# stefanch/sGDML

Measured on AMD Instinct MI355X. Metric: kernel-matrix build+solve wall-clock, N_train=1000 21-atom (aspirin-sized), lower is better.
Workload: dtype f64

## Files before the change

sgdml_amd/csrc/chol.hip:

```cpp
#include "common.h"
#include <type_traits>
#include <utility>

typedef double d4 __attribute__((ext_vector_type(4)));
typedef double d2 __attribute__((ext_vector_type(2)));

#define GT 128
#define GBK 16
#define GPITCH 17

struct GemmArgs {
  const double* A;
  const double* B;
  double* C;
  int64_t M, N, K, lda, ldb, ldc;
  int lower;
  int tiles_m, tiles_n;
  int64_t n_super;
  int64_t s_begin;
  int super_n;
  int aligned;
  int cyc_W, cyc_rank;
  int64_t cyc_lb0, cyc_nb, cyc_col0, cyc_block_rows;
  double* diagA;
  int diag_nbw;
  int64_t diag_off;
  int* diag_info;
  int col0_first;
  int* ready;
  int ready_target, ready_rows;
  const double* A2;
  const double* B2;
  double* C2;
  int64_t M2, N2, K2;
  int tiles2;
};

__global__ void __launch_bounds__(256, 2) gemm_nt_sub_diag_kernel(GemmArgs g);

template <bool FULL>
__device__ __forceinline__ void gemm_load_tile(const double* __restrict__ G, int64_t ld,
                                               int64_t row0, int64_t nrows, int64_t k0, int64_t K,
                                               int tid, d2 (&r)[4]) {
#pragma unroll
  for (int s = 0; s < 4; ++s) {
    int cidx = tid + 256 * s;
    int row = cidx >> 3, kc = (cidx & 7) * 2;
    int64_t gr = row0 + row, gk = k0 + kc;
    if (FULL) {
      r[s] = *reinterpret_cast<const d2*>(G + gr * ld + gk);
    } else {
      int64_t cr = gr < nrows ? gr : nrows - 1;
      int64_t ck0 = gk < K ? gk : K - 1, ck1 = gk + 1 < K ? gk + 1 : K - 1;
      double v0 = G[cr * ld + ck0], v1 = G[cr * ld + ck1];
      d2 v;
      v.x = (gr < nrows && gk < K) ? v0 : 0.0;
      v.y = (gr < nrows && gk + 1 < K) ? v1 : 0.0;
      r[s] = v;
    }
  }
}

__device__ __forceinline__ void gemm_load_tile_g(const double* __restrict__ base, const unsigned (&off)[4], d2 (&r)[4]) {
  typedef const __attribute__((address_space(1))) char* gcptr;
  typedef const __attribute__((address_space(1))) d2* gd2ptr;
  const uint64_t p = reinterpret_cast<uint64_t>(base);
  const uint32_t lo = __builtin_amdgcn_readfirstlane((uint32_t)p), hi = __builtin_amdgcn_readfirstlane((uint32_t)(p >> 32));
  gcptr b = (gcptr)(((uint64_t)hi << 32) | lo);
// ... 130 lines not shown
          const int64_t gr = row0 + wm * 64 + i * 16 + lk + 4 * r;
          if (gc < g.N && gr < g.M) g.C[gr * g.ldc + gc] = -acc[i][j][r];
        }
    }
    return;
  }
#pragma unroll
  for (int j = 0; j < 4; ++j) {
    double cv[4][4];
    const int64_t gc = col0 + wn * 64 + j * 16 + li;
    const bool cok = gc < g.N;
#pragma unroll
    for (int i = 0; i < 4; ++i)
#pragma unroll
      for (int r = 0; r < 4; ++r) {
        const int64_t gr = row0 + wm * 64 + i * 16 + lk + 4 * r;
        const int64_t cr = gr < g.M ? gr : g.M - 1, cc = cok ? gc : g.N - 1;
        cv[i][r] = g.C[cr * g.ldc + cc];
      }
#pragma unroll
    for (int i = 0; i < 4; ++i)
#pragma unroll
      for (int r = 0; r < 4; ++r) {
        const int64_t gr = row0 + wm * 64 + i * 16 + lk + 4 * r;
        if (cok && gr < g.M) g.C[gr * g.ldc + gc] = cv[i][r] - acc[i][j][r];
      }
  }
}

template <bool OW>
__device__ __forceinline__ void gemm_block(const GemmArgs& g, double (*lds)[2][GT * GPITCH], int64_t b) {
  if (b < g.tiles2) {
    const int tn2 = (int)((g.N2 + GT - 1) / GT);
    const int64_t ti = b / tn2, tj = b - ti * tn2;
    if (ti < tn2 && tj > ti) return;
    GemmArgs h = g;
    h.A = g.A2; h.B = g.B2; h.C = g.C2; h.M = g.M2; h.N = g.N2; h.K = g.K2;
    h.aligned = ((reinterpret_cast<uintptr_t>(g.A2) | reinterpret_cast<uintptr_t>(g.B2)) & 15) == 0 && g.aligned;
    const int64_t row0 = ti * GT, col0 = tj * GT;
    const bool full = (row0 + GT <= h.M) && (col0 + GT <= h.N) && ((h.K & (GBK - 1)) == 0) && h.aligned;
    if (full)
      gemm_tile_body<true, false>(h, lds, row0, col0);
    else
      gemm_tile_body<false, false>(h, lds, row0, col0);
    if (g.ready && ti < g.ready_rows && tj < g.ready_rows) {
      __threadfence();
      __syncthreads();
      if (threadIdx.x == 0) atomicAdd(g.ready, 1);
    }
    return;
  }
  b -= g.tiles2;
  const int64_t xcd = b & 7, loc = b >> 3;
  const int64_t s = g.s_begin + (loc >> 6) * 8 + xcd;
  const int within = (int)(loc & 63);
  if (s >= g.n_super) return;
  int64_t SI, SJ;
  if (g.lower) {
    int64_t sr = s, shift = 0;
    const int64_t sm = (g.tiles_m + 7) / 8;
    if (g.col0_first) {
      if (s < sm) { SI = s; SJ = 0; sr = -1; }
      else { sr = s - sm; shift = 1; }
    }
    if (sr >= 0) {
      SI = (int64_t)((sqrt(8.0 * (double)sr + 1.0) - 1.0) * 0.5);
      while (SI * (SI + 1) / 2 > sr) --SI;
      while ((SI + 1) * (SI + 2) / 2 <= sr) ++SI;
      SJ = sr - SI * (SI + 1) / 2;
      SI += shift; SJ += shift;
    }
  } else {
    SI = s / g.super_n;
    SJ = s - SI * g.super_n;
  }
  const int64_t ti = SI * 8 + (within >> 3), tj = SJ * 8 + (within & 7);
  if (ti >= g.tiles_m || tj >= g.tiles_n) return;
  if (g.lower && tj > ti) return;
  const int64_t row0 = ti * GT, col0 = tj * GT;
  if (g.cyc_W > 0 && row0 + GT <= g.cyc_block_rows) {
    const int64_t gb = (g.cyc_lb0 + row0 / g.cyc_nb) * g.cyc_W + g.cyc_rank;
    const int64_t grow_last = gb * g.cyc_nb + (row0 + GT - 1) % g.cyc_nb;
    if (g.cyc_col0 + col0 > grow_last) return;
  }
  const bool full = (row0 + GT <= g.M) && (col0 + GT <= g.N) && ((g.K & (GBK - 1)) == 0) && g.aligned;
  if (full)
    gemm_tile_body<true, OW>(g, lds, row0, col0);
  else
    gemm_tile_body<false, OW>(g, lds, row0, col0);
  if (g.ready && g.tiles2 == 0 && ti < g.ready_rows && tj < g.ready_rows) {
    __threadfence();
    __syncthreads();
    if (threadIdx.x == 0) atomicAdd(g.ready, 1);
  }
}

__global__ void __launch_bounds__(256, 2) gemm_nt_sub_kernel(GemmArgs g) {
  __shared__ __attribute__((aligned(16))) double lds[2][2][GT * GPITCH];
  gemm_block<false>(g, lds, blockIdx.x);
}


__global__ void __launch_bounds__(256, 2) gemm_nt_neg_kernel(GemmArgs g) {
  __shared__ __attribute__((aligned(16))) double lds[2][2][GT * GPITCH];
  gemm_block<true>(g, lds, blockIdx.x);
}

struct DiagJob {
  double* A = nullptr;
  int nbw = 0;
  int64_t off = 0;
  int* ready = nullptr;
  int ready_target = 0;
  bool col0_first = false;
  const double* A2 = nullptr;
  const double* B2 = nullptr;
  double* C2 = nullptr;
  int64_t M2 = 0, N2 = 0, K2 = 0;
};

static int launch_gemm_nt_sub_part(gdml_ctx* ctx, hipStream_t st, const double* A, int64_t lda,
                                   const double* B, int64_t ldb, double* C, int64_t ldc, int64_t M,
                                   int64_t N, int64_t K, int lower, double f0, double f1, bool timed,
                                   const DiagJob* diag = nullptr, const CyclicLower* cyc = nullptr, bool overwrite = false) {
  if (M <= 0 || N <= 0 || K <= 0) return GDML_OK;
  GemmArgs g;
  g.A = A; g.B = B; g.C = C; g.M = M; g.N = N; g.K = K; g.lda = lda; g.ldb = ldb; g.ldc = ldc;
  g.lower = lower;
  g.diagA = nullptr; g.diag_nbw = 0; g.diag_off = 0; g.diag_info = nullptr;
  g.cyc_W = 0; g.cyc_rank = 0; g.cyc_lb0 = 0; g.cyc_nb = 0; g.cyc_col0 = 0; g.cyc_block_rows = 0;
  g.col0_first = (diag && diag->col0_first) ? 1 : 0;
  g.ready = nullptr; g.ready_target = 0; g.ready_rows = 0;
  g.A2 = g.B2 = nullptr; g.C2 = nullptr; g.M2 = g.N2 = g.K2 = 0; g.tiles2 = 0;
  if (cyc) { g.cyc_W = cyc->W; g.cyc_rank = cyc->rank; g.cyc_lb0 = cyc->lb0; g.cyc_nb = cyc->nb; g.cyc_col0 = cyc->col0; g.cyc_block_rows = cyc->block_rows; }
  g.aligned = ((reinterpret_cast<uintptr_t>(A) | reinterpret_cast<uintptr_t>(B)) & 15) == 0 &&
              (lda % 2 == 0) && (ldb % 2 == 0);
  g.tiles_m = (int)((M + GT - 1) / GT);
  g.tiles_n = (int)((N + GT - 1) / GT);
  int64_t sm = (g.tiles_m + 7) / 8, sn = (g.tiles_n + 7) / 8;
  g.super_n = (int)sn;
  const int64_t n_super_all = lower ? sm * (sm + 1) / 2 : sm * sn;
  g.s_begin = (int64_t)(f0 * (double)n_super_all);
  g.n_super = (f1 >= 1.0) ? n_super_all : (int64_t)(f1 * (double)n_super_all);
  const bool has_diag = diag && diag->A;
  if (g.n_super <= g.s_begin) {
    if (!has_diag) return GDML_OK;
    g.n_super = g.s_begin;
  }
  int64_t groups = (g.n_super - g.s_begin + 7) / 8;
  int64_t blocks = groups * 512;
  const int slot = (timed && st == (ctx->kt_stream ? ctx->kt_stream : ctx->stream)) ? ktime_begin(ctx) : -1;
  if (has_diag) {
    g.diagA = diag->A; g.diag_nbw = diag->nbw; g.diag_off = diag->off; g.diag_info = ctx->d_info;
    if (diag->ready) { g.ready = diag->ready; g.ready_target = diag->ready_target; g.ready_rows = diag->nbw * 64 / GT; }
    if (diag->A2 && diag->M2 > 0) {
      g.A2 = diag->A2; g.B2 = diag->B2; g.C2 = diag->C2; g.M2 = diag->M2; g.N2 = diag->N2; g.K2 = diag->K2;
      g.tiles2 = (int)(ceil_div(g.M2, GT) * ceil_div(g.N2, GT));
    }
    hipLaunchKernelGGL(gemm_nt_sub_diag_kernel, dim3((unsigned)(blocks + 1 + g.tiles2)), dim3(256), 0, st, g);
  } else if (overwrite)
    hipLaunchKernelGGL(gemm_nt_neg_kernel, dim3((unsigned)blocks), dim3(256), 0, st, g);
  else
    hipLaunchKernelGGL(gemm_nt_sub_kernel, dim3((unsigned)blocks), dim3(256), 0, st, g);
  const double part = (double)(g.n_super - g.s_begin) / (double)n_super_all;
  ktime_end(ctx, slot, has_diag ? "gemm_nt_sub_diag" : "gemm_nt_sub",
            part * (lower ? (double)M * (double)(M + 1) * (double)K : 2.0 * (double)M * (double)N * (double)K) +
                2.0 * (double)g.M2 * (double)g.N2 * (double)g.K2);
  ctx->launch_counter++;
  HIP_CHECK(ctx, hipGetLastError());
  return GDML_OK;
}

int launch_gemm_nt_sub(gdml_ctx* ctx, hipStream_t st, const double* A, int64_t lda,
                              const double* B, int64_t ldb, double* C, int64_t ldc, int64_t M,
                              int64_t N, int64_t K, int lower) {
  return launch_gemm_nt_sub_part(ctx, st, A, lda, B, ldb, C, ldc, M, N, K, lower, 0.0, 1.0, true);
}

int launch_gemm_nt_neg(gdml_ctx* ctx, hipStream_t st, const double* A, int64_t lda, const double* B, int64_t ldb,
                       double* C, int64_t ldc, int64_t M, int64_t N, int64_t K) {
  return launch_gemm_nt_sub_part(ctx, st, A, lda, B, ldb, C, ldc, M, N, K, 0, 0.0, 1.0, true, nullptr, nullptr, true);
}

int launch_gemm_nt_sub_cyclic(gdml_ctx* ctx, hipStream_t st, const double* A, int64_t lda, const double* B, int64_t ldb,
                              double* C, int64_t ldc, int64_t M, int64_t N, int64_t K, const CyclicLower& cyc) {
  return launch_gemm_nt_sub_part(ctx, st, A, lda, B, ldb, C, ldc, M, N, K, 0, 0.0, 1.0, true, nullptr, &cyc);
}

__device__ __forceinline__ double readlane_f64(double v, int l) {
  const int lo = __builtin_amdgcn_readlane(__double2loint(v), l);
  const int hi = __builtin_amdgcn_readlane(__double2hiint(v), l);
  return __hiloint2double(hi, lo);
}
__device__ __forceinline__ int potrf64_wave(double* T, double* cb , int lane) {
  double row[64];
#pragma unroll
  for (int c = 0; c < 64; ++c) row[c] = T[lane * 65 + c];
  int fail = 0;
#pragma unroll
  for (int jb = 0; jb < 8; ++jb) {
// ... 734 lines not shown
  if (min_rows < 1) min_rows = 1;
  int64_t OB = (int64_t)ctx_opt(ctx, "chol.outer", 1024);
  if (OB != 2 * NB || NB % GT != 0) OB = NB;
  const int64_t outer_min_rows = (int64_t)ctx_opt(ctx, "chol.outer_min_rows", 16384);
  auto width_at = [&](int64_t c0) -> int64_t {
    const int64_t left = n - (c0 + OB);
    const int64_t w = (OB > NB && left > 0 && left >= outer_min_rows) ? OB : NB;
    return (n - c0 < w) ? n - c0 : w;
  };
  int64_t k0 = 0, nb = (n < NB) ? n : NB;
  int ready_count = 0;
  HIP_CHECK(ctx, hipMemsetAsync(ctx->d_info + 6, 0, 2 * sizeof(int), ctx->stream));
  GDML_TRY(panel_factor(ctx, st, A, n_rows, ld, 0, nb));
  for (;;) {
    const int64_t t0 = k0 + nb;
    if (t0 >= n) break;
    const int64_t nb2 = width_at(t0);
    const int64_t t1 = t0 + nb2;
    const double* P = A + t0 * ld + k0;
    const bool fuse = (nb2 % 64 == 0) && (n - t1 >= min_rows) && (n_rows - t1 > 0);
    if (fuse && nb2 == 2 * NB) {
      const int64_t ta = t0 + NB;
      const int64_t sm = (ceil_div(n_rows - t0, GT) + 7) / 8, n_super_all = sm * (sm + 1) / 2;
      int64_t s_split = n_super_all / 2;
      if (s_split < sm) s_split = sm;
      const double fs = ((double)s_split + 0.5) / (double)n_super_all;
      DiagJob dj;
      dj.A = A + t0 * ld + t0; dj.nbw = (int)(NB / 64); dj.off = t0;
      dj.col0_first = true;
      dj.ready = ctx->d_info + 6;
      const int block_tiles = (int)((NB / GT) * (NB / GT + 1) / 2);
      ready_count += block_tiles;
      dj.ready_target = ready_count;
      GDML_TRY(launch_gemm_nt_sub_part(ctx, st, P, ld, P, ld, A + t0 * ld + t0, ld, n_rows - t0, n - t0, nb, 1, 0.0, fs, true,
                                       &dj));
      double* Xa = A + ta * ld + t0;
      GDML_TRY(launch_panel_trsm(ctx, st, A + t0 * ld + t0, Xa, ld, (int)NB, n_rows - ta));
      dj.A = A + ta * ld + ta; dj.off = ta;
      dj.A2 = Xa; dj.B2 = Xa; dj.C2 = A + ta * ld + ta; dj.M2 = n_rows - ta; dj.N2 = NB; dj.K2 = NB;
      ready_count += block_tiles;
      dj.ready_target = ready_count;
      GDML_TRY(launch_gemm_nt_sub_part(ctx, st, P, ld, P, ld, A + t0 * ld + t0, ld, n_rows - t0, n - t0, nb, 1, fs, 1.0, true,
                                       &dj));
      GDML_TRY(launch_panel_trsm(ctx, st, A + ta * ld + ta, A + t1 * ld + ta, ld, (int)NB, n_rows - t1));
    } else {
      GDML_TRY(launch_gemm_nt_sub(ctx, st, P, ld, P, ld, A + t0 * ld + t0, ld, n_rows - t0, nb2, nb, 0));
      const double* P1 = A + t1 * ld + k0;
      if (fuse) {
        DiagJob dj;
        dj.A = A + t0 * ld + t0;
        dj.nbw = (int)(nb2 / 64);
        dj.off = t0;
        GDML_TRY(launch_gemm_nt_sub_part(ctx, st, P1, ld, P1, ld, A + t1 * ld + t1, ld, n_rows - t1, n - t1, nb, 1, 0.0,
                                         1.0, true, &dj));
        GDML_TRY(launch_panel_trsm(ctx, st, A + t0 * ld + t0, A + t1 * ld + t0, ld, (int)nb2, n_rows - t1));
      } else if (t1 < n) {
        hipStream_t sp = ctx->stream2;
        HIP_CHECK(ctx, hipEventRecord(ctx->ev_la[0], st));
        HIP_CHECK(ctx, hipStreamWaitEvent(sp, ctx->ev_la[0], 0));
        GDML_TRY(panel_factor(ctx, sp, A, n_rows, ld, t0, nb2));
        HIP_CHECK(ctx, hipEventRecord(ctx->ev_la[1], sp));
        GDML_TRY(launch_gemm_nt_sub(ctx, st, P1, ld, P1, ld, A + t1 * ld + t1, ld, n_rows - t1, n - t1, nb, 1));
        HIP_CHECK(ctx, hipStreamWaitEvent(st, ctx->ev_la[1], 0));
      } else {
        GDML_TRY(panel_factor(ctx, st, A, n_rows, ld, t0, nb2));
      }
// ... 340 lines not shown
```

sgdml_amd/csrc/common.h:

```cpp
#pragma once
#include <hip/hip_runtime.h>
#include <stdint.h>
#include <stdio.h>
#include <stdlib.h>
#include <string.h>

#include <map>
#include <string>
#include <vector>

#include "../../include/gdml_hip.h"

#define GDML_MAX_ATOMS 4096

struct Lattice {
  double lat[9];
  double inv[9];
  int use;
};

struct PhaseStat {
  double ms = 0.0;
  int64_t launches = 0;
};
// ... 26 lines not shown
  std::vector<int32_t> h_tp, h_perm, h_pinv;
};

struct Model {
  int64_t M = 0;
  int N = 0, D = 0, P = 0;
  double sig = 0;
  double* xp = nullptr;
  double* jap = nullptr;
  double* ja = nullptr;
  double* aE = nullptr;
  int32_t* tp = nullptr;
  bool has_aE = false;
};

enum CtxSlot {
  SLOT_PREDICT_WS = 0,
  SLOT_MATVEC_OUT = 1,
  SLOT_LEV_SCORES = 2,
  SLOT_PRECON_GEMV = 3,
  SLOT_PREDICT_STATS = 4,
  SLOT_PANEL_SAVE = 5,
  SLOT_LU_UT = 6,
  SLOT_WIDE_WS = 7,
  SLOT_PANEL_TRSM = 8,
  SLOT_WIDE_PARTS = 9,
  SLOT_PRECON_MF = 10,
  SLOT_F32_GRAM_ROWS = 11,
  SLOT_MATVEC_VREF = 12,
  SLOT_GRAM_WS = 13,
  SLOT_GRAM_ROWS = 14,
  SLOT_COUNT
};

struct gdml_ctx {
  int device = 0;
  int num_cus = 256;
  hipStream_t stream = nullptr;
  hipStream_t stream2 = nullptr;
  hipStream_t kt_stream = nullptr;
  hipEvent_t ev0 = nullptr, ev1 = nullptr;
  hipEvent_t ev_la[6] = {};
  std::string err;
  std::map<std::string, double> opts;
  int64_t held = 0;
  std::map<void*, int64_t> allocs;
  std::map<std::string, PhaseStat> phases;
  std::string phase_pending;
  int64_t phase_pending_launches = 0;
  double* h_pin = nullptr;
  int64_t h_pin_bytes = 0;
  double* h_map = nullptr;
  double* h_map_dev = nullptr;
  unsigned* d_fused_counter = nullptr;
  unsigned long long fused_seq = 0;
  int64_t launch_counter = 0;
  bool profiling = false;
  std::map<std::string, KernelStat> kstats;
  std::vector<PendingTiming> pending;
  std::vector<hipEvent_t> event_pool;

  TrainSet ts;
  Model model;

  double* K = nullptr;
  int64_t K_rows = 0, K_cols = 0, K_extra = 0, K_ld = 0, K_bytes = 0;
  bool K_factored = false;
  bool K_destroyed = false;
  bool K_is_A = false;
  bool K_rhs_row = false;
  double* d_rhs = nullptr;
  double K_lam = 0, K_sig = 0;
  bool uncert_ready = false;
  int K_use_E = 0;

  double* precon = nullptr;
  int64_t precon_m = 0, precon_n = 0;
  int precon_form = 0, precon_stage = 2, precon_use_E = 0;
  double precon_sig = 0;
  double* precon_Z = nullptr;
  int64_t precon_Z_bytes = 0;
  int64_t* precon_idx = nullptr;
  int64_t precon_idx_bytes = 0;
  float* precon_X32 = nullptr;
  int64_t precon_X32_bytes = 0;
  bool precon_X32_inplace = false;
  int64_t precon_X32_ld = 0;
  std::vector<double> precon_lev_cache;
  double* precon_T0 = nullptr;
  int64_t precon_T0_bytes = 0;

  double* scratch = nullptr;
  int64_t scratch_bytes = 0;
  double* slot[SLOT_COUNT] = {};
  int64_t slot_bytes[SLOT_COUNT] = {};
  int* d_info = nullptr;

  void* comm = nullptr;
  void* comm2 = nullptr;
  int rank = 0, world = 1;
  struct {
    bool on = false;
    void *comm = nullptr, *comm2 = nullptr;
    int rank = 0, world = 1;
    bool virtual_rank = false;
    gdml_host_allreduce ar = nullptr;
    gdml_host_allgather ag = nullptr;
  } parked;
  bool virtual_rank = false;
  gdml_host_allreduce host_allreduce = nullptr;
  bool comm_aborted = false;
  gdml_host_allgather host_allgather = nullptr;
  void* host_coll_user = nullptr;
  double* h_coll = nullptr;
  int64_t h_coll_bytes = 0;
  int64_t coll_calls = 0;
  double coll_bytes = 0.0;
  bool K_sharded = false;
  int64_t K_rows_global = 0;
};

int gdml_fail(gdml_ctx* ctx, int code, const char* fmt, ...);
double ctx_opt(const gdml_ctx* ctx, const char* key, double dflt);
static inline int ctx_opt_i(const gdml_ctx* ctx, const char* key, int dflt) { return (int)ctx_opt(ctx, key, (double)dflt); }

#define HIP_CHECK(ctx, call)                                                              \
  do {                                                                                    \
    hipError_t e__ = (call);                                                              \
    if (e__ != hipSuccess)                                                                \
// ... 36 lines not shown

int desc_device(gdml_ctx* ctx, const double* d_R, int64_t M, int N, const double* lat,
                const double* lat_inv, double* d_x, double* d_g);
int predict_device(gdml_ctx* ctx, const double* d_xq, const double* d_gq, int64_t B, double* d_E,
                   double* d_F);
int hess_device(gdml_ctx* ctx, const double* d_xq, const double* d_gq, int64_t B, double* d_E, double* d_F,
                double* d_H);
int predict_wide_device(gdml_ctx* ctx, const double* d_xq, int64_t B, double* part_F, double* part_E);
int set_alphas_device(gdml_ctx* ctx, const double* d_alphas_F, const double* d_alphas_E);
int matvec_device(gdml_ctx* ctx, double lam, int use_E_cstr, const double* d_v, int64_t n,
                  double* d_out);
int chol_factor_device(gdml_ctx* ctx, double* A, int64_t n, int64_t ld, int* info, int64_t n_rows = 0);
int lu_factor_device(gdml_ctx* ctx, double* A, int64_t n, int64_t ld, int64_t* d_piv, int* info_out);
int chol_solve_device(gdml_ctx* ctx, const double* L, int64_t n, int64_t ld, double* d_b,
                      double* d_z, double* d_x);
int operator_model_from_trainset(gdml_ctx* ctx, double sig);
int launch_gemm_nt_sub(gdml_ctx* ctx, hipStream_t st, const double* A, int64_t lda, const double* B,
                       int64_t ldb, double* C, int64_t ldc, int64_t M, int64_t N, int64_t K, int lower);
int launch_gemm_nt_neg(gdml_ctx* ctx, hipStream_t st, const double* A, int64_t lda, const double* B, int64_t ldb,
                       double* C, int64_t ldc, int64_t M, int64_t N, int64_t K);
struct CyclicLower {
  int W = 0, rank = 0;
  int64_t lb0 = 0, nb = 0, col0 = 0, block_rows = 0;
};
int launch_gemm_nt_sub_cyclic(gdml_ctx* ctx, hipStream_t st, const double* A, int64_t lda, const double* B, int64_t ldb,
                              double* C, int64_t ldc, int64_t M, int64_t N, int64_t K, const CyclicLower& cyc);
int launch_trsm64(gdml_ctx* ctx, hipStream_t st, const double* Ld, double* X, int64_t ld, int w,
                  int64_t m, int64_t ldl = 0);
int launch_panel_trsm(gdml_ctx* ctx, hipStream_t st, const double* L, double* X, int64_t ld, int nb, int64_t m,
                      int64_t ldl = 0);
int panel_factor_steps(gdml_ctx* ctx, hipStream_t st, double* A, int64_t n, int64_t ld, int64_t k0, int64_t nb);
int chol_bwd_device(gdml_ctx* ctx, const double* L, int64_t n, int64_t ld, double* d_z, double* d_x);
int tall_trsm(gdml_ctx* ctx, const double* L, double* X, int64_t n, int64_t m, int64_t ld, int look = -1);
int ctx_slot(gdml_ctx* ctx, int slot, int64_t bytes, double** out);
int ctx_slot_release(gdml_ctx* ctx, int slot);
struct GramSplit {
  int n3, nblk, npairs, S;
  int64_t n, ld, L;
};
GramSplit gram_split(int64_t n, int n3);
static inline int64_t pad_rows128(int64_t rows) { return (rows + 127) / 128 * 128; }
int gram_workspace(gdml_ctx* ctx, const GramSplit& g, const char* chunk_opt, int64_t items, int64_t ws_per_item, int64_t ws_fixed,
                   int64_t* chunk, double** rows, double** ws);
void block_gram_launch(gdml_ctx* ctx, const GramSplit& g, const double* Z, double* part, int64_t items, bool diag, int64_t first0,
                       int64_t first_stride, int64_t pitch = 0);
int cross_rows_launch(gdml_ctx* ctx, const double* xt, const double* gt, int64_t M, const double* xq, const double* gq, int bc,
                      double* rows, int64_t ld, double* kqq, double sgn, double sig, const char* tname);
void cov_reduce_launch(gdml_ctx* ctx, const GramSplit& g, const double* part, const double* nkqq, double* out, int64_t items,
                       int full);
void shard_points(const gdml_ctx* ctx, int64_t M, int64_t* p0, int64_t* p1, int64_t* pts_per);
struct VecLayout {
  int64_t n = 0, n_ff = 0, M = 0, N3 = 0, per = 0;
  int64_t chunk = 0, n_pad = 0, row0 = 0, n_loc = 0;
  int two_seg = 0;
  __host__ __device__ int64_t pos(int64_t g) const {
    if (!two_seg) return g;
    if (g < n_ff) {
      const int64_t pt = g / N3, r = pt / per;
      return r * chunk + (pt - r * per) * N3 + (g - pt * N3);
    }
    const int64_t e = g - n_ff, r = e / per;
    const int64_t cnt = (M - r * per < per) ? M - r * per : per;
    return r * chunk + cnt * N3 + (e - r * per);
  }
};
VecLayout vec_layout(const gdml_ctx* ctx, int use_E_cstr);
// ... 11 lines not shown
```

sgdml_amd/csrc/ctx.hip:

```cpp
#include <stdarg.h>

#include <mutex>

#include "common.h"

static std::string g_create_err;

int gdml_fail(gdml_ctx* ctx, int code, const char* fmt, ...) {
  char buf[1024];
  va_list ap;
  va_start(ap, fmt);
  vsnprintf(buf, sizeof(buf), fmt, ap);
  va_end(ap);
  if (ctx)
    ctx->err = buf;
  else
    g_create_err = buf;
  return code;
}

extern "C" int gdml_abi_version(void) { return 4; }

static const char* kKnownOptions[] = {
    "asm.wave", "asm.j_chunk", "asm.lower", "asm.strip", "asm.i_chunk",
    "asm.pts", "asm.pts_nv", "asm.pts_nt", "asm.pts_xcd", "asm.pts_i_chunk", "asm.pts_debug", "asm.perm_debug", "asm.perm_w", "asm.perm_lds_kb", "asm.perm_level", "asm.perm_nimg", "asm.perm_pg", "asm.perm_na", "asm.perm_fast_store", "asm.perm_i_chunk", "asm.perm_compact", "asm.perm_lds_rows", "asm.big1", "asm.perm2", "asm.perm2_min_n", "asm.perm2_min_p", "asm.perm2_split", "asm.perm2_post", "asm.perm2_ed", "asm.perm2_es", "asm.perm2_direct", "asm.perm2_chunk", "asm.perm2_i_chunk", "asm.perm2_debug",
    "nys.trsm_left", "nys.syrk_split", "predict.wide_pad", "predict.tn_fill", "chol.nb", "pcg.gemv_plain",
    "chol.fused_min_rows", "chol.outer", "chol.outer_min_rows", "trsm.debug",
    "trsv.persist", "predict.wave_only", "predict.mfma", "predict.fill", "predict.mfma_wide", "predict.fused", "predict.fused_rows", "predict.fused_spin",
    "lu.nb", "comm.force_collectives", "nys.force_qr", "nys.force_fail", "dist.nb", "dist.lookahead", "dist.force_panels", "pcg.depth", "pcg.precon_form", "pcg.f32_rows_per", "pcg.f32_rw", "pcg.f32_min_pivot", "pcg.f32_last_min_pivot", "pcg.f32_gram_rows", "pcg.f32_inplace",
    "predict.hess_generic", "predict.hess_chunk_rows", "predict.cov_chunk", "predict.cov_global", "predict.cov_few_rows", "predict.cov_few_split_timers", "chol.loo_chunk", "chol.extend_chunk", "chol.remove_chunk", "chol.select_chunk", "chol.select_mem_budget",
    "chol.evidence_chunk", "chol.evidence_mem_budget", "chol.evidence_global"};

double ctx_opt(const gdml_ctx* ctx, const char* key, double dflt) {
  auto it = ctx->opts.find(key);
  return it == ctx->opts.end() ? dflt : it->second;
}

extern "C" int gdml_set_option(gdml_ctx* ctx, const char* key, double value) {
  if (!ctx || !key) return GDML_ERR_INVALID;
  for (const char* k : kKnownOptions)
    if (strcmp(k, key) == 0) {
      ctx->opts[key] = value;
      return GDML_OK;
    }
  return gdml_fail(ctx, GDML_ERR_INVALID, "gdml_set_option: unknown option '%s'", key);
}

extern "C" int gdml_get_option(gdml_ctx* ctx, const char* key, double* value_out, int* is_set_out) {
  if (!ctx || !key) return GDML_ERR_INVALID;
  auto it = ctx->opts.find(key);
  if (value_out) *value_out = it == ctx->opts.end() ? 0.0 : it->second;
  if (is_set_out) *is_set_out = it != ctx->opts.end();
  return GDML_OK;
}

static void options_from_env(gdml_ctx* ctx) {
  const char* e = getenv("GDML_OPTIONS");
  if (!e) return;
  std::string s(e);
  size_t pos = 0;
// ... 114 lines not shown
      (e = hipEventCreateWithFlags(&ctx->ev_la[1], hipEventDisableTiming)) != hipSuccess ||
      (e = hipEventCreateWithFlags(&ctx->ev_la[2], hipEventDisableTiming)) != hipSuccess ||
      (e = hipEventCreateWithFlags(&ctx->ev_la[3], hipEventDisableTiming)) != hipSuccess ||
      (e = hipEventCreateWithFlags(&ctx->ev_la[4], hipEventDisableTiming)) != hipSuccess ||
      (e = hipEventCreateWithFlags(&ctx->ev_la[5], hipEventDisableTiming)) != hipSuccess ||
      (e = hipMalloc((void**)&ctx->d_info, 64)) != hipSuccess) {
    gdml_fail(nullptr, GDML_ERR_HIP, "context setup failed: %s", hipGetErrorString(e));
    delete ctx;
    return GDML_ERR_HIP;
  }
  options_from_env(ctx);
  *ctx_out = ctx;
  return GDML_OK;
}

extern "C" int gdml_ctx_destroy(gdml_ctx* ctx) {
  if (!ctx) return GDML_OK;
  hipSetDevice(ctx->device);
  hipDeviceSynchronize();
  comm_destroy(ctx);
  for (auto& t : ctx->pending) {
    hipEventDestroy(t.e0);
    hipEventDestroy(t.e1);
  }
  for (auto e : ctx->event_pool) hipEventDestroy(e);
  {
    std::lock_guard<std::mutex> lk(g_arena_mu);
    DeviceArena* a = arena_of(ctx);
    for (auto& kv : ctx->allocs)
      if (!arena_owns(a, kv.first)) hipFree(kv.first);
    ctx->allocs.clear();
    arena_release_owner(ctx);
  }
  if (ctx->d_info) hipFree(ctx->d_info);
  if (ctx->ev0) hipEventDestroy(ctx->ev0);
  if (ctx->ev1) hipEventDestroy(ctx->ev1);
  for (hipEvent_t ev : ctx->ev_la)
    if (ev) hipEventDestroy(ev);
  if (ctx->stream) hipStreamDestroy(ctx->stream);
  if (ctx->stream2) hipStreamDestroy(ctx->stream2);
  if (ctx->h_pin) hipHostFree(ctx->h_pin);
  if (ctx->h_map) hipHostFree(ctx->h_map);
  if (ctx->h_coll) hipHostFree(ctx->h_coll);
  delete ctx;
  return GDML_OK;
}

extern "C" const char* gdml_last_error(const gdml_ctx* ctx) {
  return ctx ? ctx->err.c_str() : g_create_err.c_str();
}

extern "C" int gdml_sync(gdml_ctx* ctx) {
  if (!ctx) return GDML_ERR_INVALID;
  HIP_CHECK(ctx, hipSetDevice(ctx->device));
  HIP_CHECK(ctx, hipStreamSynchronize(ctx->stream));
  HIP_CHECK(ctx, hipStreamSynchronize(ctx->stream2));
  return GDML_OK;
}

extern "C" int gdml_mem_info(gdml_ctx* ctx, int64_t* held, int64_t* free_b, int64_t* total_b) {
  if (!ctx) return GDML_ERR_INVALID;
  size_t f = 0, t = 0;
  HIP_CHECK(ctx, hipSetDevice(ctx->device));
  HIP_CHECK(ctx, hipMemGetInfo(&f, &t));
  if (held) *held = ctx->held;
  {
// ... 271 lines not shown
```

Before: 1.297.

## Balance lower-triangular GEMM tiles across XCDs with host-built schedule tables

Adds a host-built, cached tile schedule for the lower-triangular trailing GEMM update. Full 8x8 super-tiles are decoded arithmetically, and partial or diagonal tiles are dealt evenly across the eight XCD block slots through a small device table. The schedule accounts for second-GEMM lead work and for two-launch splits. It also packs the fused second GEMM's tiles compactly, so no blocks are launched only to exit early on upper-triangle tiles. The aim is to cut wasted empty blocks and XCD load imbalance. The cost is host-side schedule construction, plus a one-time device allocation, copy and stream sync per new shape.

After: 1.281 (median of 6 runs). 1.3% less time.

```diff
diff --git a/sgdml_amd/csrc/chol.hip b/sgdml_amd/csrc/chol.hip
--- a/sgdml_amd/csrc/chol.hip
+++ b/sgdml_amd/csrc/chol.hip
@@ -1,4 +1,6 @@
 #include "common.h"
+#include "tile_sched.h"
+#include <array>
 #include <type_traits>
 #include <utility>
 
@@ -34,6 +36,9 @@
   double* C2;
   int64_t M2, N2, K2;
   int tiles2;
+  int second_compact;
+  int bal;
+  TileLaunch tl;
 };
 
 __global__ void __launch_bounds__(256, 2) gemm_nt_sub_diag_kernel(GemmArgs g);
@@ -230,8 +235,13 @@
 __device__ __forceinline__ void gemm_block(const GemmArgs& g, double (*lds)[2][GT * GPITCH], int64_t b) {
   if (b < g.tiles2) {
     const int tn2 = (int)((g.N2 + GT - 1) / GT);
-    const int64_t ti = b / tn2, tj = b - ti * tn2;
-    if (ti < tn2 && tj > ti) return;
+    int64_t ti, tj;
+    if (g.second_compact) {
+      tile_decode_second(b, tn2, &ti, &tj);
+    } else {
+      ti = b / tn2; tj = b - ti * tn2;
+      if (ti < tn2 && tj > ti) return;
+    }
     GemmArgs h = g;
     h.A = g.A2; h.B = g.B2; h.C = g.C2; h.M = g.M2; h.N = g.N2; h.K = g.K2;
     h.aligned = ((reinterpret_cast<uintptr_t>(g.A2) | reinterpret_cast<uintptr_t>(g.B2)) & 15) == 0 && g.aligned;
@@ -249,32 +259,12 @@
     return;
   }
   b -= g.tiles2;
-  const int64_t xcd = b & 7, loc = b >> 3;
-  const int64_t s = g.s_begin + (loc >> 6) * 8 + xcd;
-  const int within = (int)(loc & 63);
-  if (s >= g.n_super) return;
-  int64_t SI, SJ;
-  if (g.lower) {
-    int64_t sr = s, shift = 0;
-    const int64_t sm = (g.tiles_m + 7) / 8;
-    if (g.col0_first) {
-      if (s < sm) { SI = s; SJ = 0; sr = -1; }
-      else { sr = s - sm; shift = 1; }
-    }
-    if (sr >= 0) {
-      SI = (int64_t)((sqrt(8.0 * (double)sr + 1.0) - 1.0) * 0.5);
-      while (SI * (SI + 1) / 2 > sr) --SI;
-      while ((SI + 1) * (SI + 2) / 2 <= sr) ++SI;
-      SJ = sr - SI * (SI + 1) / 2;
-      SI += shift; SJ += shift;
-    }
-  } else {
-    SI = s / g.super_n;
-    SJ = s - SI * g.super_n;
-  }
-  const int64_t ti = SI * 8 + (within >> 3), tj = SJ * 8 + (within & 7);
-  if (ti >= g.tiles_m || tj >= g.tiles_n) return;
-  if (g.lower && tj > ti) return;
+  int64_t ti, tj;
+  if (g.bal) {
+    if (!tile_decode_bal(g.tl, b, &ti, &tj)) return;
+  } else if (!tile_decode_super(b, g.lower, g.col0_first, g.tiles_m, g.tiles_n, g.super_n, g.s_begin, g.n_super, &ti, &tj)) {
+    return;
+  }
   const int64_t row0 = ti * GT, col0 = tj * GT;
   if (g.cyc_W > 0 && row0 + GT <= g.cyc_block_rows) {
     const int64_t gb = (g.cyc_lb0 + row0 / g.cyc_nb) * g.cyc_W + g.cyc_rank;
@@ -315,7 +305,73 @@
   const double* B2 = nullptr;
   double* C2 = nullptr;
   int64_t M2 = 0, N2 = 0, K2 = 0;
+  int64_t next_M2 = 0, next_N2 = 0, next_K2 = 0;
 };
+
+struct TileSchedEntry {
+  TileSched S;
+  const uint32_t* dev[2] = {nullptr, nullptr};
+};
+struct TileSchedCache {
+  std::map<std::array<int64_t, 7>, TileSchedEntry> entries;
+  char* block = nullptr;
+  size_t cap = 0, used = 0;
+};
+
+void tile_sched_cache_free(gdml_ctx* ctx) {
+  if (!ctx->tile_sched) return;
+  if (ctx->tile_sched->block) hipFree(ctx->tile_sched->block);
+  delete ctx->tile_sched;
+  ctx->tile_sched = nullptr;
+}
+
+static int second_blocks(int64_t M2, int64_t N2, bool* compact) {
+  const int64_t tm2 = ceil_div(M2, GT), tn2 = ceil_div(N2, GT);
+  *compact = tm2 >= tn2;
+  return (int)(tm2 * tn2 - (*compact ? tn2 * (tn2 - 1) / 2 : 0));
+}
+
+static int tile_sched_get(gdml_ctx* ctx, hipStream_t st, int tiles_m, int tiles_n, bool col0_first, int n_launch, int lead2,
+                          int64_t K2, int64_t K, const TileSchedEntry** out) {
+  *out = nullptr;
+  if (!ctx->tile_sched) ctx->tile_sched = new TileSchedCache();
+  TileSchedCache* c = ctx->tile_sched;
+  const std::array<int64_t, 7> key = {tiles_m, tiles_n, col0_first ? 1 : 0, n_launch, lead2, lead2 ? K2 : 0, lead2 ? K : 0};
+  auto it = c->entries.find(key);
+  if (it == c->entries.end()) {
+    TileSchedEntry e;
+    double base[8] = {0, 0, 0, 0, 0, 0, 0, 0};
+    for (int q = 0; q < lead2; ++q) base[((q - lead2) % 8 + 8) % 8] += (double)K2 / (double)K;
+    tile_sched_build(tiles_m, tiles_n, col0_first, n_launch, base, &e.S);
+    if (e.S.ok) {
+      const size_t b0 = (e.S.table[0].size() * 4 + 255) & ~(size_t)255, b1 = (e.S.table[1].size() * 4 + 255) & ~(size_t)255;
+      const size_t block_bytes = (size_t)8 << 20;
+      if (!c->block) {
+        HIP_CHECK(ctx, hipMalloc((void**)&c->block, block_bytes));
+        c->cap = block_bytes;
+      }
+      if (b0 + b1 > c->cap) {
+        e.S.ok = false;
+      } else {
+        if (c->used + b0 + b1 > c->cap) {
+          HIP_CHECK(ctx, hipDeviceSynchronize());
+          c->entries.clear();
+          c->used = 0;
+        }
+        char* d = c->block + c->used;
+        c->used += b0 + b1;
+        if (!e.S.table[0].empty()) HIP_CHECK(ctx, hipMemcpyAsync(d, e.S.table[0].data(), e.S.table[0].size() * 4, hipMemcpyHostToDevice, st));
+        if (!e.S.table[1].empty()) HIP_CHECK(ctx, hipMemcpyAsync(d + b0, e.S.table[1].data(), e.S.table[1].size() * 4, hipMemcpyHostToDevice, st));
+        HIP_CHECK(ctx, hipStreamSynchronize(st));
+        e.dev[0] = reinterpret_cast<const uint32_t*>(d);
+        e.dev[1] = reinterpret_cast<const uint32_t*>(d + b0);
+      }
+    }
+    it = c->entries.emplace(key, std::move(e)).first;
+  }
+  if (it->second.S.ok) *out = &it->second;
+  return GDML_OK;
+}
 
 static int launch_gemm_nt_sub_part(gdml_ctx* ctx, hipStream_t st, const double* A, int64_t lda,
                                    const double* B, int64_t ldb, double* C, int64_t ldc, int64_t M,
@@ -329,7 +385,8 @@
   g.cyc_W = 0; g.cyc_rank = 0; g.cyc_lb0 = 0; g.cyc_nb = 0; g.cyc_col0 = 0; g.cyc_block_rows = 0;
   g.col0_first = (diag && diag->col0_first) ? 1 : 0;
   g.ready = nullptr; g.ready_target = 0; g.ready_rows = 0;
-  g.A2 = g.B2 = nullptr; g.C2 = nullptr; g.M2 = g.N2 = g.K2 = 0; g.tiles2 = 0;
+  g.A2 = g.B2 = nullptr; g.C2 = nullptr; g.M2 = g.N2 = g.K2 = 0; g.tiles2 = 0; g.second_compact = 0;
+  g.bal = 0; g.tl = TileLaunch();
   if (cyc) { g.cyc_W = cyc->W; g.cyc_rank = cyc->rank; g.cyc_lb0 = cyc->lb0; g.cyc_nb = cyc->nb; g.cyc_col0 = cyc->col0; g.cyc_block_rows = cyc->block_rows; }
   g.aligned = ((reinterpret_cast<uintptr_t>(A) | reinterpret_cast<uintptr_t>(B)) & 15) == 0 &&
               (lda % 2 == 0) && (ldb % 2 == 0);
@@ -341,19 +398,45 @@
   g.s_begin = (int64_t)(f0 * (double)n_super_all);
   g.n_super = (f1 >= 1.0) ? n_super_all : (int64_t)(f1 * (double)n_super_all);
   const bool has_diag = diag && diag->A;
-  if (g.n_super <= g.s_begin) {
-    if (!has_diag) return GDML_OK;
-    g.n_super = g.s_begin;
-  }
-  int64_t groups = (g.n_super - g.s_begin + 7) / 8;
-  int64_t blocks = groups * 512;
+  const bool second = has_diag && diag->A2 && diag->M2 > 0;
+  const TileSchedEntry* te = nullptr;
+  const int tl_i = f0 > 0.0 ? 1 : 0;
+  if (lower && !cyc && !overwrite && ctx_opt(ctx, "gemm.balance", 1) != 0) {
+    const int64_t M2s = second ? diag->M2 : (diag ? diag->next_M2 : 0), N2s = second ? diag->N2 : (diag ? diag->next_N2 : 0);
+    const int64_t K2s = second ? diag->K2 : (diag ? diag->next_K2 : 0);
+    bool compact = false;
+    const int lead2 = (M2s > 0 && N2s > 0) ? second_blocks(M2s, N2s, &compact) : 0;
+    GDML_TRY(tile_sched_get(ctx, st, g.tiles_m, g.tiles_n, g.col0_first != 0, (f0 > 0.0 || f1 < 1.0) ? 2 : 1, compact ? lead2 : 0,
+                            K2s, K, &te));
+  }
+  int64_t blocks;
+  if (te) {
+    g.bal = 1;
+    g.tl = te->S.L[tl_i];
+    g.tl.table = te->dev[tl_i];
+    g.s_begin = g.n_super = 0;
+    blocks = te->S.blocks[tl_i];
+    if (blocks == 0 && !has_diag) return GDML_OK;
+  } else {
+    if (g.n_super <= g.s_begin) {
+      if (!has_diag) return GDML_OK;
+      g.n_super = g.s_begin;
+    }
+    const int64_t groups = (g.n_super - g.s_begin + 7) / 8;
+    blocks = groups * 512;
+  }
   const int slot = (timed && st == (ctx->kt_stream ? ctx->kt_stream : ctx->stream)) ? ktime_begin(ctx) : -1;
   if (has_diag) {
     g.diagA = diag->A; g.diag_nbw = diag->nbw; g.diag_off = diag->off; g.diag_info = ctx->d_info;
     if (diag->ready) { g.ready = diag->ready; g.ready_target = diag->ready_target; g.ready_rows = diag->nbw * 64 / GT; }
-    if (diag->A2 && diag->M2 > 0) {
+    if (second) {
       g.A2 = diag->A2; g.B2 = diag->B2; g.C2 = diag->C2; g.M2 = diag->M2; g.N2 = diag->N2; g.K2 = diag->K2;
       g.tiles2 = (int)(ceil_div(g.M2, GT) * ceil_div(g.N2, GT));
+      if (te) {
+        bool compact = false;
+        const int lead2 = second_blocks(g.M2, g.N2, &compact);
+        if (compact) { g.tiles2 = lead2; g.second_compact = 1; }
+      }
     }
     hipLaunchKernelGGL(gemm_nt_sub_diag_kernel, dim3((unsigned)(blocks + 1 + g.tiles2)), dim3(256), 0, st, g);
   } else if (overwrite)
@@ -361,9 +444,9 @@
   else
     hipLaunchKernelGGL(gemm_nt_sub_kernel, dim3((unsigned)blocks), dim3(256), 0, st, g);
   const double part = (double)(g.n_super - g.s_begin) / (double)n_super_all;
-  ktime_end(ctx, slot, has_diag ? "gemm_nt_sub_diag" : "gemm_nt_sub",
-            part * (lower ? (double)M * (double)(M + 1) * (double)K : 2.0 * (double)M * (double)N * (double)K) +
-                2.0 * (double)g.M2 * (double)g.N2 * (double)g.K2);
+  const double flops = te ? tile_sched_flops(te->S, tl_i, M, K, g.tiles_m, GT)
+                          : part * (lower ? (double)M * (double)(M + 1) * (double)K : 2.0 * (double)M * (double)N * (double)K);
+  ktime_end(ctx, slot, has_diag ? "gemm_nt_sub_diag" : "gemm_nt_sub", flops + 2.0 * (double)g.M2 * (double)g.N2 * (double)g.K2);
   ctx->launch_counter++;
   HIP_CHECK(ctx, hipGetLastError());
   return GDML_OK;
@@ -1164,6 +1247,7 @@
       const int block_tiles = (int)((NB / GT) * (NB / GT + 1) / 2);
       ready_count += block_tiles;
       dj.ready_target = ready_count;
+      dj.next_M2 = n_rows - ta; dj.next_N2 = NB; dj.next_K2 = NB;
       GDML_TRY(launch_gemm_nt_sub_part(ctx, st, P, ld, P, ld, A + t0 * ld + t0, ld, n_rows - t0, n - t0, nb, 1, 0.0, fs, true,
                                        &dj));
       double* Xa = A + ta * ld + t0;
diff --git a/sgdml_amd/csrc/common.h b/sgdml_amd/csrc/common.h
--- a/sgdml_amd/csrc/common.h
+++ b/sgdml_amd/csrc/common.h
@@ -82,6 +82,8 @@
   SLOT_GRAM_ROWS = 14,
   SLOT_COUNT
 };
+
+struct TileSchedCache;
 
 struct gdml_ctx {
   int device = 0;
@@ -145,6 +147,7 @@
   double* slot[SLOT_COUNT] = {};
   int64_t slot_bytes[SLOT_COUNT] = {};
   int* d_info = nullptr;
+  TileSchedCache* tile_sched = nullptr;
 
   void* comm = nullptr;
   void* comm2 = nullptr;
@@ -247,6 +250,7 @@
 int panel_factor_steps(gdml_ctx* ctx, hipStream_t st, double* A, int64_t n, int64_t ld, int64_t k0, int64_t nb);
 int chol_bwd_device(gdml_ctx* ctx, const double* L, int64_t n, int64_t ld, double* d_z, double* d_x);
 int tall_trsm(gdml_ctx* ctx, const double* L, double* X, int64_t n, int64_t m, int64_t ld, int look = -1);
+void tile_sched_cache_free(gdml_ctx* ctx);
 int ctx_slot(gdml_ctx* ctx, int slot, int64_t bytes, double** out);
 int ctx_slot_release(gdml_ctx* ctx, int slot);
 struct GramSplit {
diff --git a/sgdml_amd/csrc/ctx.hip b/sgdml_amd/csrc/ctx.hip
--- a/sgdml_amd/csrc/ctx.hip
+++ b/sgdml_amd/csrc/ctx.hip
@@ -25,7 +25,7 @@
     "asm.wave", "asm.j_chunk", "asm.lower", "asm.strip", "asm.i_chunk",
     "asm.pts", "asm.pts_nv", "asm.pts_nt", "asm.pts_xcd", "asm.pts_i_chunk", "asm.pts_debug", "asm.perm_debug", "asm.perm_w", "asm.perm_lds_kb", "asm.perm_level", "asm.perm_nimg", "asm.perm_pg", "asm.perm_na", "asm.perm_fast_store", "asm.perm_i_chunk", "asm.perm_compact", "asm.perm_lds_rows", "asm.big1", "asm.perm2", "asm.perm2_min_n", "asm.perm2_min_p", "asm.perm2_split", "asm.perm2_post", "asm.perm2_ed", "asm.perm2_es", "asm.perm2_direct", "asm.perm2_chunk", "asm.perm2_i_chunk", "asm.perm2_debug",
     "nys.trsm_left", "nys.syrk_split", "predict.wide_pad", "predict.tn_fill", "chol.nb", "pcg.gemv_plain",
-    "chol.fused_min_rows", "chol.outer", "chol.outer_min_rows", "trsm.debug",
+    "chol.fused_min_rows", "chol.outer", "chol.outer_min_rows", "gemm.balance", "trsm.debug",
     "trsv.persist", "predict.wave_only", "predict.mfma", "predict.fill", "predict.mfma_wide", "predict.fused", "predict.fused_rows", "predict.fused_spin",
     "lu.nb", "comm.force_collectives", "nys.force_qr", "nys.force_fail", "dist.nb", "dist.lookahead", "dist.force_panels", "pcg.depth", "pcg.precon_form", "pcg.f32_rows_per", "pcg.f32_rw", "pcg.f32_min_pivot", "pcg.f32_last_min_pivot", "pcg.f32_gram_rows", "pcg.f32_inplace",
     "predict.hess_generic", "predict.hess_chunk_rows", "predict.cov_chunk", "predict.cov_global", "predict.cov_few_rows", "predict.cov_few_split_timers", "chol.loo_chunk", "chol.extend_chunk", "chol.remove_chunk", "chol.select_chunk", "chol.select_mem_budget",
@@ -206,6 +206,7 @@
     ctx->allocs.clear();
     arena_release_owner(ctx);
   }
+  tile_sched_cache_free(ctx);
   if (ctx->d_info) hipFree(ctx->d_info);
   if (ctx->ev0) hipEventDestroy(ctx->ev0);
   if (ctx->ev1) hipEventDestroy(ctx->ev1);
diff --git a/sgdml_amd/csrc/tile_sched.h b/sgdml_amd/csrc/tile_sched.h
--- /dev/null
+++ b/sgdml_amd/csrc/tile_sched.h
@@ -0,0 +1,258 @@
+#pragma once
+#include <math.h>
+#include <stdint.h>
+#include <vector>
+
+#if defined(__HIPCC__)
+#define TS_HD __host__ __device__ __forceinline__
+#else
+#define TS_HD inline
+#endif
+
+TS_HD void ts_tri(int64_t t, int64_t* I, int64_t* J) {
+  int64_t i = (int64_t)((sqrt(8.0 * (double)t + 1.0) - 1.0) * 0.5);
+  while (i * (i + 1) / 2 > t) --i;
+  while ((i + 1) * (i + 2) / 2 <= t) ++i;
+  *I = i;
+  *J = t - i * (i + 1) / 2;
+}
+
+TS_HD bool tile_decode_super(int64_t b, int lower, int col0_first, int tiles_m, int tiles_n, int super_n, int64_t s_begin,
+                             int64_t n_super, int64_t* ti_out, int64_t* tj_out) {
+  const int64_t xcd = b & 7, loc = b >> 3;
+  const int64_t s = s_begin + (loc >> 6) * 8 + xcd;
+  const int within = (int)(loc & 63);
+  if (s >= n_super) return false;
+  int64_t SI = 0, SJ = 0;
+  if (lower) {
+    int64_t sr = s, shift = 0;
+    const int64_t sm = (tiles_m + 7) / 8;
+    if (col0_first) {
+      if (s < sm) { SI = s; SJ = 0; sr = -1; }
+      else { sr = s - sm; shift = 1; }
+    }
+    if (sr >= 0) {
+      ts_tri(sr, &SI, &SJ);
+      SI += shift; SJ += shift;
+    }
+  } else {
+    SI = s / super_n;
+    SJ = s - SI * super_n;
+  }
+  const int64_t ti = SI * 8 + (within >> 3), tj = SJ * 8 + (within & 7);
+  if (ti >= tiles_m || tj >= tiles_n) return false;
+  if (lower && tj > ti) return false;
+  *ti_out = ti; *tj_out = tj;
+  return true;
+}
+
+struct TileLaunch {
+  const uint32_t* table;
+  int stride;
+  int r0, r1;
+  int nh;
+  int col0_first;
+  uint64_t hn[2], tn[2];
+};
+
+TS_HD int ts_unpack(const uint64_t (&w)[2], int x) { return (int)((w[x >> 2] >> (16 * (x & 3))) & 0xffff); }
+
+TS_HD void ts_full_super(int64_t f, int col0_first, int nh, int64_t* SI, int64_t* SJ) {
+  if (col0_first) {
+    if (f < nh) { *SI = f + 1; *SJ = 0; return; }
+    ts_tri(f - nh, SI, SJ);
+    *SI += 2; *SJ += 1;
+  } else {
+    ts_tri(f, SI, SJ);
+    *SI += 1;
+  }
+}
+
+TS_HD bool tile_decode_bal(const TileLaunch& L, int64_t b, int64_t* ti, int64_t* tj) {
+  const int x = (int)(b & 7);
+  const int64_t pos = b >> 3;
+  const int hn = ts_unpack(L.hn, x);
+  const int64_t q = pos - hn, full_slots = (int64_t)(L.r1 - L.r0) * 64;
+  if (q >= 0 && q < full_slots) {
+    int64_t SI, SJ;
+    ts_full_super(((int64_t)L.r0 + (q >> 6)) * 8 + x, L.col0_first, L.nh, &SI, &SJ);
+    *ti = SI * 8 + ((q & 63) >> 3);
+    *tj = SJ * 8 + (q & 7);
+    return true;
+  }
+  int64_t e = pos;
+  if (q >= 0) {
+    e = q - full_slots;
+    if (e >= ts_unpack(L.tn, x)) return false;
+    e += hn;
+  }
+  uint32_t v = L.table[(int64_t)x * L.stride + e];
+#if defined(__HIP_DEVICE_COMPILE__)
+  v = __builtin_amdgcn_readfirstlane(v);
+#endif
+  *ti = v & 0xffff;
+  *tj = v >> 16;
+  return true;
+}
+
+TS_HD void tile_decode_second(int64_t b, int tn2, int64_t* ti, int64_t* tj) {
+  const int64_t nlow = (int64_t)tn2 * (tn2 + 1) / 2;
+  if (b < nlow) { ts_tri(b, ti, tj); return; }
+  const int64_t r = b - nlow;
+  *ti = tn2 + r / tn2;
+  *tj = r % tn2;
+}
+
+
+struct TileSched {
+  bool ok = false;
+  int n_launch = 1;
+  TileLaunch L[2] = {};
+  std::vector<uint32_t> table[2];
+  int64_t blocks[2] = {0, 0};
+  int64_t tiles[2] = {0, 0};
+  int64_t off_int[2] = {0, 0}, off_last[2] = {0, 0}, diag_int[2] = {0, 0}, diag_last[2] = {0, 0};
+};
+
+namespace ts_detail {
+struct Deal { std::vector<uint32_t> t[8]; };
+
+inline void deal(const std::vector<uint32_t>& tiles, const int64_t prior[8], const double base[8], Deal* d) {
+  int64_t total = (int64_t)tiles.size();
+  for (int x = 0; x < 8; ++x) total += prior[x];
+  const int64_t q = total / 8;
+  int rem = (int)(total % 8);
+  int64_t want[8];
+  bool extra[8] = {};
+  for (int x = 0; x < 8; ++x)
+    if (prior[x] > q && rem > 0) { extra[x] = true; --rem; }
+  while (rem > 0) {
+    int best = -1;
+    for (int x = 0; x < 8; ++x)
+      if (!extra[x] && (best < 0 || base[x] < base[best])) best = x;
+    extra[best] = true; --rem;
+  }
+  int64_t given = 0;
+  for (int x = 0; x < 8; ++x) {
+    want[x] = q + (extra[x] ? 1 : 0) - prior[x];
+    if (want[x] < 0) want[x] = 0;
+  }
+  for (int x = 0; x < 8; ++x) {
+    int64_t w = want[x];
+    if (x == 7 || w > (int64_t)tiles.size() - given) w = (int64_t)tiles.size() - given;
+    d->t[x].assign(tiles.begin() + given, tiles.begin() + given + w);
+    given += w;
+  }
+}
+}
+
+inline void tile_sched_build(int tiles_m, int tiles_n, bool col0_first, int n_launch, const double base_last[8], TileSched* S) {
+  *S = TileSched();
+  S->n_launch = n_launch;
+  const int sm = (tiles_m + 7) / 8, fm = tiles_m / 8;
+  if (tiles_m < 1 || tiles_n < 1 || tiles_n > tiles_m || tiles_m > 0xffff || (n_launch != 1 && n_launch != 2)) return;
+  if (fm >= 2 && (fm - 1) * 8 > tiles_n) return;
+  const int nh = col0_first ? (fm > 1 ? fm - 1 : 0) : 0;
+  const int64_t F = (int64_t)fm * (fm - 1) / 2, R = F / 8;
+  std::vector<uint32_t> head, tail;
+  int64_t f = 0, total = R * 512;
+  auto visit = [&](int SI, int SJ) {
+    const bool full = SI < fm && SJ < SI;
+    if (full && f++ < R * 8) return;
+    std::vector<uint32_t>& v = (col0_first && SJ == 0) ? head : tail;
+    for (int r = 0; r < 8; ++r)
+      for (int c = 0; c < 8; ++c) {
+        const int ti = SI * 8 + r, tj = SJ * 8 + c;
+        if (ti < tiles_m && tj < tiles_n && tj <= ti) { v.push_back((uint32_t)ti | ((uint32_t)tj << 16)); ++total; }
+      }
+  };
+  if (col0_first) {
+    for (int SI = 1; SI < fm; ++SI) visit(SI, 0);
+    std::vector<uint32_t> rest;
+    rest.swap(head);
+    visit(0, 0);
+    head.insert(head.end(), rest.begin(), rest.end());
+    for (int SI = fm > 1 ? fm : 1; SI < sm; ++SI) visit(SI, 0);
+    for (int SI = 1; SI < sm; ++SI)
+      for (int SJ = 1; SJ <= SI; ++SJ) visit(SI, SJ);
+  } else {
+    for (int SI = 0; SI < sm; ++SI)
+      for (int SJ = 0; SJ <= SI; ++SJ) visit(SI, SJ);
+  }
+  int64_t r_cut = R;
+  if (n_launch == 2) {
+    r_cut = (int64_t)floor(((double)total * 0.5 - (double)head.size()) / 512.0 + 0.5);
+    const int64_t need = (((int64_t)nh < R * 8 ? (int64_t)nh : R * 8) + 7) / 8;
+    if (r_cut < need) r_cut = need;
+    if (r_cut > R) r_cut = R;
+  }
+  const int64_t zero[8] = {0, 0, 0, 0, 0, 0, 0, 0};
+  const double nobase[8] = {0, 0, 0, 0, 0, 0, 0, 0};
+  ts_detail::Deal dh, dt, dl;
+  ts_detail::deal(head, zero, nobase, &dh);
+  std::vector<uint32_t> tail_last, tail_rest;
+  for (uint32_t v : tail) ((int)(v & 0xffff) == tiles_m - 1 ? tail_last : tail_rest).push_back(v);
+  int64_t prior[8];
+  for (int x = 0; x < 8; ++x) prior[x] = (n_launch == 1) ? (int64_t)dh.t[x].size() : 0;
+  ts_detail::deal(tail_last, prior, nobase, &dl);
+  for (int x = 0; x < 8; ++x) prior[x] += (int64_t)dl.t[x].size();
+  ts_detail::deal(tail_rest, prior, base_last ? base_last : nobase, &dt);
+  for (int x = 0; x < 8; ++x) dt.t[x].insert(dt.t[x].begin(), dl.t[x].begin(), dl.t[x].end());
+  const int last = n_launch - 1;
+  for (int l = 0; l < n_launch; ++l) {
+    TileLaunch& L = S->L[l];
+    L.table = nullptr;
+    L.r0 = (l == 0) ? 0 : (int)r_cut;
+    L.r1 = (l == last) ? (int)R : (int)r_cut;
+    L.nh = nh;
+    L.col0_first = col0_first ? 1 : 0;
+    int64_t per[8], mx = 0, cnt_max = 0;
+    for (int x = 0; x < 8; ++x) {
+      const int64_t h = (l == 0) ? (int64_t)dh.t[x].size() : 0, t = (l == last) ? (int64_t)dt.t[x].size() : 0;
+      if (h > 0xffff || t > 0xffff) return;
+      L.hn[x >> 2] |= (uint64_t)h << (16 * (x & 3));
+      L.tn[x >> 2] |= (uint64_t)t << (16 * (x & 3));
+      per[x] = h + t;
+      if (per[x] > mx) mx = per[x];
+      const int64_t c = per[x] + (int64_t)(L.r1 - L.r0) * 64;
+      if (c > cnt_max) cnt_max = c;
+    }
+    L.stride = (int)mx;
+    S->table[l].assign((size_t)(8 * mx), 0);
+    for (int x = 0; x < 8; ++x) {
+      size_t o = (size_t)x * (size_t)mx;
+      if (l == 0) for (uint32_t v : dh.t[x]) S->table[l][o++] = v;
+      if (l == last) for (uint32_t v : dt.t[x]) S->table[l][o++] = v;
+    }
+    S->blocks[l] = 8 * cnt_max;
+    auto count = [&](int64_t ti, int64_t tj) {
+      const bool lastrow = ti == tiles_m - 1;
+      ++S->tiles[l];
+      if (ti == tj) ++(lastrow ? S->diag_last[l] : S->diag_int[l]);
+      else ++(lastrow ? S->off_last[l] : S->off_int[l]);
+    };
+    for (int x = 0; x < 8; ++x) {
+      if (l == 0) for (uint32_t v : dh.t[x]) count(v & 0xffff, v >> 16);
+      if (l == last) for (uint32_t v : dt.t[x]) count(v & 0xffff, v >> 16);
+    }
+    for (int64_t ff = (int64_t)L.r0 * 8; ff < (int64_t)L.r1 * 8; ++ff) {
+      int64_t SI, SJ;
+      ts_full_super(ff, L.col0_first, L.nh, &SI, &SJ);
+      for (int r = 0; r < 8; ++r)
+        for (int c = 0; c < 8; ++c) count(SI * 8 + r, SJ * 8 + c);
+    }
+  }
+  S->ok = true;
+}
+
+inline double tile_sched_counted_flops(const TileSched& S, int l, int64_t M, int64_t K, int tiles_m, int gt) {
+  const double rl = (double)(M - (int64_t)(tiles_m - 1) * gt), g = (double)gt;
+  return (double)K * (2.0 * g * g * (double)S.off_int[l] + 2.0 * rl * g * (double)S.off_last[l] +
+                      g * (g + 1.0) * (double)S.diag_int[l] + rl * (rl + 1.0) * (double)S.diag_last[l]);
+}
+inline double tile_sched_flops(const TileSched& S, int l, int64_t M, int64_t K, int tiles_m, int gt) {
+  if (l < S.n_launch - 1) return tile_sched_counted_flops(S, l, M, K, tiles_m, gt);
+  double before = 0.0;
+  for (int i = 0; i < l; ++i) before += tile_sched_counted_flops(S, i, M, K, tiles_m, gt);
+  return (double)M * (double)(M + 1) * (double)K - before;
+}
```
